# patflick/psac

Hardware: AMD Instinct MI355X
Metric: MChars/s SA+LCP build; rank-pair radix-sort HBM GB/s vs peak (higher is better)
Workload: dtype u64

## Files before the change

include/psacx.h:

```cpp
#ifndef PSACX_H
#define PSACX_H

#include <stddef.h>
#include <stdint.h>

#ifdef __cplusplus
extern "C" {
#endif

typedef struct psacx_ctx psacx_ctx;

enum {
    PSACX_OK = 0,
    PSACX_EINVAL = -1,
    PSACX_ERANGE = -2,
    PSACX_ENOMEM = -3,
    PSACX_EHIP = -4,
    PSACX_EDEVICE = -5,
    PSACX_ENOGPU = -6
};

enum {
    PSACX_LCP = 1u,
    PSACX_NO_FAST = 2u,
// ... 15 lines not shown
    uint32_t sigma;
    uint32_t bits_per_char;
    uint32_t k;
    uint32_t n_rounds;
    psacx_round rounds[PSACX_MAX_ROUNDS];
    double ms_total;
    double ms_alphabet, ms_kmer, ms_sort_hist, ms_sort_scatter, ms_rebucket, ms_isa_scatter,
           ms_gather, ms_compact, ms_rmq_build, ms_finalize;
    double ms_sort_scatter3, ms_sort_tilehist, ms_sort_scatter2;
    uint64_t scatter_launches[3];
    uint64_t scatter_records[3];
    uint64_t scatter_bytes[3];
    uint64_t hist_bytes;
    uint64_t workspace_bytes;
    uint64_t onew_passes;
    uint64_t heavy_rounds;
    uint64_t heavy_records;
    uint64_t light_records;
    uint64_t level_gathers;
    double ms_host[9];
    uint64_t locate_fetches[2];
    uint64_t rebucket_1w;
    uint64_t group_sort;
    uint64_t grid_cuts;
} psacx_stats;


#define PSACX_STREAM_DEFAULT ((void*)(intptr_t)-1)
int psacx_create(psacx_ctx** out, int device, void* stream);
void psacx_destroy(psacx_ctx* ctx);
const char* psacx_strerror(int code);
const char* psacx_last_hip_error(const psacx_ctx* ctx);
int psacx_trim(psacx_ctx* ctx);

enum {
    PSACX_OPT_RESET = 0, PSACX_OPT_FORCE_DIET, PSACX_OPT_DIET_CAP, PSACX_OPT_ONE_STAGE, PSACX_OPT_TIES_RADIX, PSACX_OPT_NO_ONE_WORD,
    PSACX_OPT_ONE_WORD_ALWAYS, PSACX_OPT_ONE_WORD_MIN, PSACX_OPT_WIDEN_LAST, PSACX_OPT_NO_DIGIT_BYTES, PSACX_OPT_NO_BUCKET_SORT,
    PSACX_OPT_ISA_UPDATE, PSACX_OPT_GATHER, PSACX_OPT_NO_HEAVY, PSACX_OPT_NO_WHOLE, PSACX_OPT_NO_LAZY_RANKS, PSACX_OPT_NO_EARLY_OUT,
    PSACX_OPT_NO_SPREAD_CURSORS, PSACX_OPT_LOCATE_SHAPE, PSACX_OPT_LOCATE_COUNT, PSACX_OPT_GENERIC_REBUCKET,
    PSACX_OPT_PLAIN_SIDE_KERNELS, PSACX_OPT_LSD_BUCKET_PASSES, PSACX_OPT_FIRST_LEAD, PSACX_OPT_LZ_SMALL_TILES,
    PSACX_OPT_GRID_CAP, PSACX_OPT_GROUP_COUNTING_ROUNDS, PSACX_OPT_MEMS_STOP, PSACX_OPT_KMISMATCH_STOP,
    PSACX_OPT_KEDIT_STOP,
    PSACX_OPT_COUNT
};
int psacx_configure(psacx_ctx* ctx, int option, uint64_t value);
int psacx_configure_from_env(psacx_ctx* ctx);
const char* psacx_debug_env(const char* name);

int psacx_construct_u32(psacx_ctx* ctx, const uint8_t* text, uint64_t n, uint32_t k,
                        uint32_t flags, uint32_t* SA, uint32_t* ISA, uint32_t* LCP);
int psacx_construct_u64(psacx_ctx* ctx, const uint8_t* text, uint64_t n, uint32_t k,
                        uint32_t flags, uint64_t* SA, uint64_t* ISA, uint64_t* LCP);
int psacx_construct_dev_u32(psacx_ctx* ctx, const uint8_t* d_text, uint64_t n, uint32_t k,
                            uint32_t flags, uint32_t* d_SA, uint32_t* d_ISA, uint32_t* d_LCP);
int psacx_construct_dev_u64(psacx_ctx* ctx, const uint8_t* d_text, uint64_t n, uint32_t k,
                            uint32_t flags, uint64_t* d_SA, uint64_t* d_ISA, uint64_t* d_LCP);

int psacx_construct_lc_u32(psacx_ctx* ctx, const uint8_t* text, uint64_t n, uint32_t k, uint32_t flags,
                           uint32_t* SA, uint32_t* ISA, uint32_t* LCP, uint8_t* Lc);
int psacx_construct_lc_u64(psacx_ctx* ctx, const uint8_t* text, uint64_t n, uint32_t k, uint32_t flags,
                           uint64_t* SA, uint64_t* ISA, uint64_t* LCP, uint8_t* Lc);
int psacx_construct_lc_dev_u32(psacx_ctx* ctx, const uint8_t* d_text, uint64_t n, uint32_t k, uint32_t flags,
                               uint32_t* d_SA, uint32_t* d_ISA, uint32_t* d_LCP, uint8_t* d_Lc);
int psacx_construct_lc_dev_u64(psacx_ctx* ctx, const uint8_t* d_text, uint64_t n, uint32_t k, uint32_t flags,
                               uint64_t* d_SA, uint64_t* d_ISA, uint64_t* d_LCP, uint8_t* d_Lc);

// ... 379 lines not shown
```

psac_amd/_lib.py:

```python
import ctypes as C
import os

_HERE = os.path.dirname(os.path.abspath(__file__))
LIB_PATH = os.path.join(_HERE, "lib", "libpsacx.so")

PSACX_LCP = 1
PSACX_NO_FAST = 2
PSACX_PROFILE = 4
PSACX_MAX_ROUNDS = 72
PSACX_MATCH_SUFFIXES = 1
PSACX_OVERLAP_WHOLE = 1
PSACX_REPEATS_RIGHT, PSACX_REPEATS_MAXIMAL, PSACX_REPEATS_SUPERMAXIMAL = 0, 1, 2
PSACX_MEMS_SUPER = 1
PSACX_KEDIT_BEST = 1

OPTIONS = {"reset": 0, "force_diet": 1, "diet_cap": 2, "one_stage": 3, "ties_radix": 4, "no_one_word": 5, "one_word_always": 6, "one_word_min": 7,
           "widen_last": 8, "no_digit_bytes": 9, "no_bucket_sort": 10, "isa_update": 11, "gather": 12, "no_heavy": 13, "no_whole": 14, "no_lazy_ranks": 15, "no_early_out": 16,
           "no_spread_cursors": 17, "locate_shape": 18, "locate_count": 19, "generic_rebucket": 20,
           "plain_side_kernels": 21, "lsd_bucket_passes": 22, "first_lead": 23, "lz_small_tiles": 24,
           "grid_cap": 25}
KERNEL_OPTIONS = {"group_counting_rounds": 26, "mems_stop": 27, "kmismatch_stop": 28, "kedit_stop": 29}
MULTI_OPTIONS = {"layout": 1, "slab": 2, "output_slack": 3, "trace": 4, "wire_piece": 5, "pieces": 6, "check_chunks": 7, "global_refine_sort": 8,
                 "one_stage": 9, "two_word": 10, "one_word": 11, "no_slices": 12, "slice_wide": 13, "slice_shape": 14}
MULTI_FORCE_WIRE, MULTI_NO_RCCL, MULTI_SHM = 1, 2, 4
ENV_KNOBS = bool(os.environ.get("PSACX_ENV_KNOBS"))
if ENV_KNOBS and os.environ.get("PSACX_LIB"):
    LIB_PATH = os.environ["PSACX_LIB"]

EXPORTS = [
    "psacx_create", "psacx_destroy", "psacx_strerror", "psacx_last_hip_error", "psacx_trim", "psacx_configure", "psacx_configure_from_env", "psacx_debug_env",
    "psacx_construct_u32", "psacx_construct_u64", "psacx_construct_dev_u32", "psacx_construct_dev_u64",
    "psacx_construct_gsa_u32", "psacx_construct_gsa_u64", "psacx_construct_gsa_dev_u32", "psacx_construct_gsa_dev_u64",
    "psacx_construct_lc_u32", "psacx_construct_lc_u64", "psacx_construct_lc_dev_u32", "psacx_construct_lc_dev_u64",
    "psacx_get_stats", "psacx_profile", "psacx_check_dev_u32", "psacx_check_dev_u64", "psacx_check_gsa_dev_u32", "psacx_check_gsa_dev_u64", "psacx_pair_sort_dev_u32", "psacx_pair_sort_dev_u64", "psacx_ansv_u32",
    "psacx_ansv_u64", "psacx_ansv_dev_u32", "psacx_ansv_dev_u64", "psacx_suffix_tree_u32", "psacx_suffix_tree_u64", "psacx_suffix_tree_dev_u32", "psacx_suffix_tree_dev_u64",
    "psacx_check_suffix_tree_dev_u32", "psacx_check_suffix_tree_dev_u64",
    "psacx_suffix_tree_gsa_u32", "psacx_suffix_tree_gsa_u64", "psacx_suffix_tree_gsa_dev_u32", "psacx_suffix_tree_gsa_dev_u64",
    "psacx_check_suffix_tree_gsa_dev_u32", "psacx_check_suffix_tree_gsa_dev_u64", "psacx_dev_alloc", "psacx_dev_free", "psacx_copy_h2d", "psacx_copy_d2h", "psacx_sync",
    "psacx_rand_dna", "psacx_synth_text_dev",
    "psacx_lookup_table_dev_u32", "psacx_lookup_table_dev_u64", "psacx_locate_dev_u32", "psacx_locate_dev_u64", "psacx_locate_u32", "psacx_locate_u64",
    "psacx_string_ends_dev", "psacx_lookup_table_gsa_dev_u32", "psacx_lookup_table_gsa_dev_u64", "psacx_locate_gsa_dev_u32", "psacx_locate_gsa_dev_u64",
    "psacx_locate_gsa_u32", "psacx_locate_gsa_u64", "psacx_occurrences_dev_u32", "psacx_occurrences_dev_u64",
    "psacx_match_dev_u32", "psacx_match_dev_u64", "psacx_match_gsa_dev_u32", "psacx_match_gsa_dev_u64",
    "psacx_match_u32", "psacx_match_u64", "psacx_match_gsa_u32", "psacx_match_gsa_u64",
# ... 18 lines not shown
    "psacx_multi_left_chars_dev_u32", "psacx_multi_left_chars_dev_u64", "psacx_multi_construct_lc_u32", "psacx_multi_construct_lc_u64",
    "psacx_multi_configure", "psacx_multi_configure_from_env", "psacx_multi_create_ex", "psacx_multi_create_rank_ex", "psacx_multi_get_memory", "psacx_multi_transport", "psacx_multi_get_wire", "psacx_multi_get_phases", "psacx_multi_last_form",
]


class Round(C.Structure):
    _fields_ = [("h", C.c_uint64), ("active", C.c_uint64), ("unfinished_buckets", C.c_uint64),
                ("unfinished_elements", C.c_uint64), ("sort_passes", C.c_uint32),
                ("sort_passes_skipped", C.c_uint32)]


class Stats(C.Structure):
    _fields_ = [("sigma", C.c_uint32), ("bits_per_char", C.c_uint32), ("k", C.c_uint32),
                ("n_rounds", C.c_uint32), ("rounds", Round * PSACX_MAX_ROUNDS),
                ("ms_total", C.c_double), ("ms_alphabet", C.c_double), ("ms_kmer", C.c_double),
                ("ms_sort_hist", C.c_double), ("ms_sort_scatter", C.c_double), ("ms_rebucket", C.c_double),
                ("ms_isa_scatter", C.c_double), ("ms_gather", C.c_double), ("ms_compact", C.c_double),
                ("ms_rmq_build", C.c_double), ("ms_finalize", C.c_double),
                ("ms_sort_scatter3", C.c_double), ("ms_sort_tilehist", C.c_double), ("ms_sort_scatter2", C.c_double),
                ("scatter_launches", C.c_uint64 * 3), ("scatter_records", C.c_uint64 * 3),
                ("scatter_bytes", C.c_uint64 * 3), ("hist_bytes", C.c_uint64), ("workspace_bytes", C.c_uint64), ("onew_passes", C.c_uint64),
                ("heavy_rounds", C.c_uint64), ("heavy_records", C.c_uint64), ("light_records", C.c_uint64), ("level_gathers", C.c_uint64),
                ("ms_host", C.c_double * 9), ("locate_fetches", C.c_uint64 * 2), ("rebucket_1w", C.c_uint64),
                ("group_sort", C.c_uint64), ("grid_cuts", C.c_uint64)]


class PsacxError(RuntimeError):
    def __init__(self, code, msg):
        RuntimeError.__init__(self, "psacx error %d: %s" % (code, msg))
        self.code = code


_lib = None


def load():
    global _lib
    if _lib is not None:
        return _lib
    if not os.path.exists(LIB_PATH):
        raise ImportError("libpsacx.so not built (%s); run `python -c 'import __graft_entry__ as g; g.build()'`"
                          % LIB_PATH)
    try:
        import torch
    except ImportError:
        pass
    lib = C.CDLL(LIB_PATH, mode=C.RTLD_GLOBAL)
# ... 150 lines not shown
```

psac_amd/csrc/dev_common.hpp:

```cpp
#pragma once
#include <hip/hip_runtime.h>
#include <stdint.h>

namespace psacx {

constexpr int WAVE = 64;

__device__ __forceinline__ unsigned lane_id() {
    return __builtin_amdgcn_mbcnt_hi(~0u, __builtin_amdgcn_mbcnt_lo(~0u, 0u));
}
__device__ __forceinline__ uint64_t lanemask_lt() {
    return (1ull << lane_id()) - 1ull;
}

template <typename T> __device__ __forceinline__ T shfl(T v, int src);
template <> __device__ __forceinline__ uint32_t shfl<uint32_t>(uint32_t v, int src) {
    return (uint32_t)__shfl((int)v, src, WAVE);
}
template <> __device__ __forceinline__ uint64_t shfl<uint64_t>(uint64_t v, int src) {
    uint32_t lo = (uint32_t)__shfl((int)(uint32_t)v, src, WAVE);
    uint32_t hi = (uint32_t)__shfl((int)(uint32_t)(v >> 32), src, WAVE);
    return ((uint64_t)hi << 32) | lo;
}
template <typename T> __device__ __forceinline__ T shfl_up(T v, int d);
// ... 13 lines not shown
    return (uint32_t)__shfl_xor((int)v, m, WAVE);
}
template <> __device__ __forceinline__ uint64_t shfl_xor<uint64_t>(uint64_t v, int m) {
    uint32_t lo = (uint32_t)__shfl_xor((int)(uint32_t)v, m, WAVE);
    uint32_t hi = (uint32_t)__shfl_xor((int)(uint32_t)(v >> 32), m, WAVE);
    return ((uint64_t)hi << 32) | lo;
}

__device__ __forceinline__ unsigned xcc_id() {
    return (unsigned)__builtin_amdgcn_s_getreg((3 << 11) | (0 << 6) | 20) & 7u;
}

__device__ __forceinline__ unsigned claim_tile(unsigned* qcnt, unsigned ntiles, unsigned chunk) {
    if (chunk == 0) return atomicAdd(qcnt, 1u);
    const unsigned x = xcc_id();
    for (unsigned r = 0; r < 8; ++r) {
        const unsigned q = (x + r) & 7u;
        const unsigned k = atomicAdd(&qcnt[q], 1u);
        const unsigned long long tile = ((unsigned long long)(k / chunk) * 8u + q) * chunk + k % chunk;
        if (tile < ntiles) return (unsigned)tile;
    }
    return ntiles;
}

struct OpSum {
    template <typename T> __device__ __forceinline__ T operator()(T a, T b) const { return a + b; }
};
struct OpMax {
    template <typename T> __device__ __forceinline__ T operator()(T a, T b) const { return a > b ? a : b; }
};
struct OpOr {
    template <typename T> __device__ __forceinline__ T operator()(T a, T b) const { return a | b; }
};
struct OpAnd {
    template <typename T> __device__ __forceinline__ T operator()(T a, T b) const { return a & b; }
};
struct OpMin {
    template <typename T> __device__ __forceinline__ T operator()(T a, T b) const { return a < b ? a : b; }
};

template <typename T, typename Op>
__device__ __forceinline__ T wave_reduce(T v, Op op) {
#pragma unroll
    for (int m = 32; m >= 1; m >>= 1) v = op(v, shfl_xor<T>(v, m));
    return v;
}
// ... 6 lines not shown
        T o = shfl_up<T>(v, d);
        if (lane >= (unsigned)d) v = op(o, v);
    }
    return v;
}

template <int BLOCK, typename T, typename Op>
__device__ __forceinline__ T block_scan_exclusive(T v, Op op, T identity, T* smem, T* total) {
    constexpr int NW = BLOCK / WAVE;
    const unsigned lane = lane_id();
    const unsigned wave = threadIdx.x / WAVE;
    T inc = wave_scan_inclusive<T>(v, op);
    if (lane == WAVE - 1) smem[wave] = inc;
    __syncthreads();
    T wprefix = identity;
    T tot = identity;
#pragma unroll
    for (int w = 0; w < NW; ++w) {
        T s = smem[w];
        if ((unsigned)w < wave) wprefix = op(wprefix, s);
        tot = op(tot, s);
    }
    T prev = shfl_up<T>(inc, 1);
    T excl = (lane == 0) ? wprefix : op(wprefix, prev);
    *total = tot;
    __syncthreads();
    return excl;
}

template <int BLOCK, typename T, typename Op>
__device__ __forceinline__ T block_reduce(T v, Op op, T* smem) {
    constexpr int NW = BLOCK / WAVE;
    v = wave_reduce<T>(v, op);
    if (lane_id() == 0) smem[threadIdx.x / WAVE] = v;
    __syncthreads();
    T r = smem[0];
#pragma unroll
    for (int w = 1; w < NW; ++w) r = op(r, smem[w]);
    __syncthreads();
    return r;
}

template <typename D> struct Desc;
template <> struct Desc<uint64_t> {
    static constexpr int SHIFT = 62;
    static constexpr uint64_t MASK = (1ull << 62) - 1ull;
// ... 160 lines not shown
```

psac_amd/csrc/engine.hpp:

```cpp
#pragma once
#include <hip/hip_runtime.h>

#include <algorithm>
#include <cstdio>
#include <cstdlib>
#include <cstring>
#include <condition_variable>
#include <functional>
#include <map>
#include <mutex>
#include <string>
#include <thread>
#include <sched.h>
#include <pthread.h>
#include <cctype>
#include <cstdio>
#include <vector>

#include "../../include/psacx.h"
#include "radix.hpp"
#include "sa_kernels.hpp"

namespace psacx {

// ... 7 lines not shown
namespace psacx { struct HostPool; }

namespace psacx {
struct Knobs {
    bool force_diet = false;
    uint64_t diet_cap = 0;
    bool one_stage = false;
    bool ties_radix = false;
    bool no_one_word = false;
    bool one_word_always = false;
    unsigned one_word_min = 24;
    int isa_update = 0;
    bool no_digit_bytes = false;
    bool no_bucket_sort = false;
    int gather = 0;
    bool no_heavy = false;
    bool no_early_out = false;
    bool no_lazy_ranks = false;
    bool no_whole = false;
    bool widen_last = false;
    bool no_spread_cursors = false;
    bool generic_rebucket = false;
    bool plain_side_kernels = false;
    bool lsd_bucket_passes = false;
    bool group_counting_rounds = false;
    unsigned first_lead = 0;
    bool lz_small_tiles = false;
    int locate_shape = 0;
    bool locate_count = false;
    unsigned mems_stop = 0;
    unsigned kedit_stop = 0;
    unsigned kmismatch_stop = 0;
    unsigned grid_cap = 0;
};

}

struct psacx_ctx {
    int device = 0;
    hipStream_t stream = nullptr;
    bool own_stream = false;
    char* slab = nullptr;
    size_t slab_bytes = 0;
    char* aux = nullptr;
    size_t aux_bytes = 0;
    char* pinned = nullptr;
// ... 942 lines not shown
            hipLaunchKernelGGL((top_digit_hist_kernel<uint64_t, BLOCK, ITEMS>), dim3((unsigned)ntiles), dim3(BLOCK), 0, c->stream, text, n, n_text, tab, ks, p0.tile_hist);
        else
            hipLaunchKernelGGL((top_digit_hist_waves_kernel<256>), dim3((unsigned)grid_for(c, ntiles * WAVE, 256, 5)), dim3(256), 0, c->stream, text, n, n_text, tab, ks,
                               ntiles, p0.tile_hist);
        PSACX_HIP(c, hipGetLastError());
    }
    {
        ProfScope ps(c, TC_SORT_TILEHIST);
        launch_pass_scans(c, p0, base0);
        PSACX_HIP(c, hipGetLastError());
    }
    PSACX_HIP(c, hipMemcpyAsync(sc.h_base, base0, RADIX * sizeof(unsigned long long), hipMemcpyDeviceToHost, c->stream));
    PSACX_HIP(c, hipStreamSynchronize(c->stream));
    unsigned long long* h_tabs = sc.h_base + (PIN_TABS - PIN_BASE) / sizeof(unsigned long long);
    for (int d = 0; d < RADIX; ++d) h_tabs[d] = sc.h_base[d];
    h_tabs[RADIX] = n;
    OneWordLayout lay = onew_layout<TILE>(h_tabs, ntiles);
    if (lay.need > sc.desc_bytes || lay.vtiles >= (1ull << 31)) return PSACX_RETRY_1W;
    if (view_out && dig && tie_bytes && !c->knobs.lsd_bucket_passes) lay = onew_group_layout<TILE>(lay, n, low, sc.desc_bytes);
    unsigned long long* const h_word = sc.h_base + (PIN_GROUP_WORD - PIN_BASE) / sizeof(unsigned long long);
    {
        ProfScope ps(c, TC_KMER);
        PSACX_HIP(c, hipMemsetAsync(scratch, 0, 256, c->stream));
        hipLaunchKernelGGL((key_scatter1w_kernel<BLOCK, ITEMS>), dim3((unsigned)ntiles), dim3(BLOCK), 0, c->stream, text, n, n_text, tab, ks, pad ? k0 : a, (int)(lo1 + low),
                           base0, p0.tile_hist, p0.slab_tot, p0.counter, sort_chunk_for(n, true), p0.slab_tiles, lo1 | (sfield << 16), (uint64_t)0,
                           (uint8_t*)nullptr, 0, pad);
        PSACX_HIP(c, hipGetLastError());
    }
    uint64_t* cur = nullptr;
    if (pad) PSACX_TRY(onew_bucket_passes(c, scratch, h_tabs, lay, k0, a, sa_out, sfield, low, lo1, n, &cur, view_out, dig, pad, tie_bytes, h_word));
    else PSACX_TRY(onew_bucket_passes(c, scratch, h_tabs, lay, a, k0, sa_out, sfield, low, lo1, n, &cur, view_out, dig, 0, tie_bytes, h_word));
    *s1 = cur;
    if (rs) { rs->sort_passes = (uint32_t)((low + RADIX_BITS - 1) / RADIX_BITS + 1); rs->sort_passes_skipped = 0; }
    return PSACX_OK;
}

}
```

psac_amd/csrc/psacx_abi.hip:

```cpp
#include "engine.hpp"
#include "query_calls.hpp"

namespace psacx {
int construct_dev_u32(psacx_ctx*, const uint8_t*, uint64_t, uint32_t, uint32_t, uint32_t*, uint32_t*, uint32_t*);
int construct_dev_u64(psacx_ctx*, const uint8_t*, uint64_t, uint32_t, uint32_t, uint64_t*, uint64_t*, uint64_t*);
int construct_host_u32(psacx_ctx*, const uint8_t*, uint64_t, uint32_t, uint32_t, uint32_t*, uint32_t*, uint32_t*);
int construct_gsa_host_u32(psacx_ctx*, const uint8_t*, uint64_t, const uint64_t*, uint64_t, uint32_t, uint32_t, uint32_t*, uint32_t*, uint32_t*);
int construct_gsa_dev_u32(psacx_ctx*, const uint8_t*, uint64_t, const uint64_t*, uint64_t, uint32_t, uint32_t, uint32_t*, uint32_t*, uint32_t*);
int construct_gsa_host_u64(psacx_ctx*, const uint8_t*, uint64_t, const uint64_t*, uint64_t, uint32_t, uint32_t, uint64_t*, uint64_t*, uint64_t*);
int construct_gsa_dev_u64(psacx_ctx*, const uint8_t*, uint64_t, const uint64_t*, uint64_t, uint32_t, uint32_t, uint64_t*, uint64_t*, uint64_t*);
int construct_lc_host_u32(psacx_ctx*, const uint8_t*, uint64_t, uint32_t, uint32_t, uint32_t*, uint32_t*, uint32_t*, uint8_t*);
int construct_lc_host_u64(psacx_ctx*, const uint8_t*, uint64_t, uint32_t, uint32_t, uint64_t*, uint64_t*, uint64_t*, uint8_t*);
int construct_lc_dev_u32(psacx_ctx*, const uint8_t*, uint64_t, uint32_t, uint32_t, uint32_t*, uint32_t*, uint32_t*, uint8_t*);
int construct_lc_dev_u64(psacx_ctx*, const uint8_t*, uint64_t, uint32_t, uint32_t, uint64_t*, uint64_t*, uint64_t*, uint8_t*);
int construct_host_u64(psacx_ctx*, const uint8_t*, uint64_t, uint32_t, uint32_t, uint64_t*, uint64_t*, uint64_t*);
int pair_sort_dev_u32(psacx_ctx*, uint32_t*, uint32_t*, uint32_t*, uint64_t, uint32_t);
int pair_sort_dev_u64(psacx_ctx*, uint64_t*, uint64_t*, uint64_t*, uint64_t, uint32_t);
int check_dev_u32(psacx_ctx*, const uint8_t*, uint64_t, const uint32_t*, const uint32_t*, const uint32_t*, uint64_t*);
int check_dev_u64(psacx_ctx*, const uint8_t*, uint64_t, const uint64_t*, const uint64_t*, const uint64_t*, uint64_t*);
int check_gsa_dev_u32(psacx_ctx*, const uint8_t*, uint64_t, const uint64_t*, uint64_t, const uint32_t*, const uint32_t*, const uint32_t*, uint64_t*);
int check_gsa_dev_u64(psacx_ctx*, const uint8_t*, uint64_t, const uint64_t*, uint64_t, const uint64_t*, const uint64_t*, const uint64_t*, uint64_t*);
int synth_text_dev(psacx_ctx*, uint8_t*, uint64_t, uint64_t, int, uint64_t, uint64_t);
int suffix_tree_host_u32(psacx_ctx*, const uint8_t*, uint64_t, const uint32_t*, const uint32_t*, uint64_t*, uint32_t*);
int suffix_tree_host_u64(psacx_ctx*, const uint8_t*, uint64_t, const uint64_t*, const uint64_t*, uint64_t*, uint32_t*);
// ... 84 lines not shown
    switch (option) {
    case PSACX_OPT_RESET: k = psacx::Knobs(); return PSACX_OK;
    case PSACX_OPT_FORCE_DIET: k.force_diet = value != 0; return PSACX_OK;
    case PSACX_OPT_DIET_CAP: k.diet_cap = value; return PSACX_OK;
    case PSACX_OPT_ONE_STAGE: k.one_stage = value != 0; return PSACX_OK;
    case PSACX_OPT_TIES_RADIX: k.ties_radix = value != 0; return PSACX_OK;
    case PSACX_OPT_NO_ONE_WORD: k.no_one_word = value != 0; return PSACX_OK;
    case PSACX_OPT_ONE_WORD_ALWAYS: k.one_word_always = value != 0; return PSACX_OK;
    case PSACX_OPT_ONE_WORD_MIN: if (value > 62) return PSACX_EINVAL; k.one_word_min = value ? (unsigned)std::max<uint64_t>(16, value) : 24u; return PSACX_OK;
    case PSACX_OPT_WIDEN_LAST: k.widen_last = value != 0; return PSACX_OK;
    case PSACX_OPT_NO_DIGIT_BYTES: k.no_digit_bytes = value != 0; return PSACX_OK;
    case PSACX_OPT_NO_BUCKET_SORT: k.no_bucket_sort = value != 0; return PSACX_OK;
    case PSACX_OPT_ISA_UPDATE: if (value > 2) return PSACX_EINVAL; k.isa_update = (int)value; return PSACX_OK;
    case PSACX_OPT_GATHER: if (value > 2) return PSACX_EINVAL; k.gather = (int)value; return PSACX_OK;
    case PSACX_OPT_NO_HEAVY: k.no_heavy = value != 0; return PSACX_OK;
    case PSACX_OPT_NO_WHOLE: k.no_whole = value != 0; return PSACX_OK;
    case PSACX_OPT_NO_LAZY_RANKS: k.no_lazy_ranks = value != 0; return PSACX_OK;
    case PSACX_OPT_NO_EARLY_OUT: k.no_early_out = value != 0; return PSACX_OK;
    case PSACX_OPT_NO_SPREAD_CURSORS: k.no_spread_cursors = value != 0; return PSACX_OK;
    case PSACX_OPT_LOCATE_SHAPE: if (value > 2) return PSACX_EINVAL; k.locate_shape = (int)value; return PSACX_OK;
    case PSACX_OPT_LOCATE_COUNT: k.locate_count = value != 0; return PSACX_OK;
    case PSACX_OPT_GENERIC_REBUCKET: k.generic_rebucket = value != 0; return PSACX_OK;
    case PSACX_OPT_PLAIN_SIDE_KERNELS: k.plain_side_kernels = value != 0; return PSACX_OK;
    case PSACX_OPT_LSD_BUCKET_PASSES: k.lsd_bucket_passes = value != 0; return PSACX_OK;
    case PSACX_OPT_GROUP_COUNTING_ROUNDS: k.group_counting_rounds = value != 0; return PSACX_OK;
    case PSACX_OPT_LZ_SMALL_TILES: k.lz_small_tiles = value != 0; return PSACX_OK;
    case PSACX_OPT_GRID_CAP: if (value > 65535) return PSACX_EINVAL; k.grid_cap = (unsigned)value; return PSACX_OK;
    case PSACX_OPT_MEMS_STOP: if (value > 3) return PSACX_EINVAL; k.mems_stop = (unsigned)value; return PSACX_OK;
    case PSACX_OPT_KMISMATCH_STOP: if (value > 2) return PSACX_EINVAL; k.kmismatch_stop = (unsigned)value; return PSACX_OK;
    case PSACX_OPT_KEDIT_STOP: if (value > 3) return PSACX_EINVAL; k.kedit_stop = (unsigned)value; return PSACX_OK;
    case PSACX_OPT_FIRST_LEAD: if (value > 64) return PSACX_EINVAL; k.first_lead = (unsigned)value; return PSACX_OK;
    default: return PSACX_EINVAL;
    }
}

const char* psacx_debug_env(const char* name) { return name ? getenv(name) : nullptr; }

int psacx_configure_from_env(psacx_ctx* c) {
    if (!c) return PSACX_EINVAL;
    static const struct { const char* name; int option; } flags[] = {
        {"PSACX_FORCE_DIET", PSACX_OPT_FORCE_DIET}, {"PSACX_ONE_STAGE", PSACX_OPT_ONE_STAGE}, {"PSACX_TIES_RADIX", PSACX_OPT_TIES_RADIX},
        {"PSACX_NO_ONE_WORD", PSACX_OPT_NO_ONE_WORD}, {"PSACX_ONE_WORD_ALWAYS", PSACX_OPT_ONE_WORD_ALWAYS}, {"PSACX_WIDEN_LAST", PSACX_OPT_WIDEN_LAST},
        {"PSACX_NO_DIGIT_BYTES", PSACX_OPT_NO_DIGIT_BYTES}, {"PSACX_NO_BUCKET_SORT", PSACX_OPT_NO_BUCKET_SORT}, {"PSACX_NO_HEAVY", PSACX_OPT_NO_HEAVY},
        {"PSACX_NO_WHOLE", PSACX_OPT_NO_WHOLE}, {"PSACX_NO_LAZY_RANKS", PSACX_OPT_NO_LAZY_RANKS},
        {"PSACX_NO_EARLY_OUT", PSACX_OPT_NO_EARLY_OUT}, {"PSACX_NO_SPREAD_CURSORS", PSACX_OPT_NO_SPREAD_CURSORS},
        {"PSACX_LOCATE_COUNT", PSACX_OPT_LOCATE_COUNT}, {"PSACX_GENERIC_REBUCKET", PSACX_OPT_GENERIC_REBUCKET},
        {"PSACX_PLAIN_SIDE_KERNELS", PSACX_OPT_PLAIN_SIDE_KERNELS}, {"PSACX_LSD_BUCKET_PASSES", PSACX_OPT_LSD_BUCKET_PASSES},
        {"PSACX_LZ_SMALL_TILES", PSACX_OPT_LZ_SMALL_TILES}, {"PSACX_GROUP_COUNTING_ROUNDS", PSACX_OPT_GROUP_COUNTING_ROUNDS}};
    (void)psacx_configure(c, PSACX_OPT_RESET, 0);
    for (const auto& f : flags) if (psacx_debug_env(f.name)) (void)psacx_configure(c, f.option, 1);
    if (const char* e = psacx_debug_env("PSACX_DIET_CAP")) (void)psacx_configure(c, PSACX_OPT_DIET_CAP, strtoull(e, nullptr, 10));
    if (const char* e = psacx_debug_env("PSACX_FIRST_LEAD")) (void)psacx_configure(c, PSACX_OPT_FIRST_LEAD, strtoull(e, nullptr, 10));
    if (const char* e = psacx_debug_env("PSACX_GRID_CAP")) (void)psacx_configure(c, PSACX_OPT_GRID_CAP, strtoull(e, nullptr, 10));
    if (const char* e = psacx_debug_env("PSACX_MEMS_STOP")) (void)psacx_configure(c, PSACX_OPT_MEMS_STOP, strtoull(e, nullptr, 10));
    if (const char* e = psacx_debug_env("PSACX_KMISMATCH_STOP")) (void)psacx_configure(c, PSACX_OPT_KMISMATCH_STOP, strtoull(e, nullptr, 10));
    if (const char* e = psacx_debug_env("PSACX_KEDIT_STOP")) (void)psacx_configure(c, PSACX_OPT_KEDIT_STOP, strtoull(e, nullptr, 10));
    if (const char* e = psacx_debug_env("PSACX_ONE_WORD_MIN")) (void)psacx_configure(c, PSACX_OPT_ONE_WORD_MIN, strtoull(e, nullptr, 10));
    if (const char* e = psacx_debug_env("PSACX_ISA_UPDATE")) (void)psacx_configure(c, PSACX_OPT_ISA_UPDATE, e[0] == 's' ? 1 : 2);
    if (const char* e = psacx_debug_env("PSACX_LOCATE_SHAPE")) (void)psacx_configure(c, PSACX_OPT_LOCATE_SHAPE, e[0] == 'g' ? 2 : 1);
    if (const char* e = psacx_debug_env("PSACX_GATHER")) (void)psacx_configure(c, PSACX_OPT_GATHER, e[0] == 'f' ? 1 : 2);
    return PSACX_OK;
}

int psacx_trim(psacx_ctx* c) {
    if (!c) return PSACX_EINVAL;
    PSACX_HIP(c, hipSetDevice(c->device));
    PSACX_HIP(c, hipStreamSynchronize(c->stream));
    if (c->slab) { PSACX_HIP(c, hipFree(c->slab)); c->slab = nullptr; c->slab_bytes = 0; }
    if (c->aux) { PSACX_HIP(c, hipFree(c->aux)); c->aux = nullptr; c->aux_bytes = 0; }
    if (c->io) { PSACX_HIP(c, hipFree(c->io)); c->io = nullptr; c->io_bytes = 0; }
    if (c->dstage) { PSACX_HIP(c, hipFree(c->dstage)); c->dstage = nullptr; }
// ... 173 lines not shown
```

psac_amd/csrc/radix.hpp:

```cpp
#pragma once
#include <type_traits>
#include "dev_common.hpp"
#include "sort_scratch.hpp"
#include "group_rank.hpp"

namespace psacx {


struct PassPlan {
    int n_pass;
    int word[MAX_PASSES];
    int shift[MAX_PASSES];
};

inline PassPlan make_plan(int bits1, int bits2, int lo1 = 0) {
    PassPlan p;
    p.n_pass = 0;
    for (int w = 1; w >= 0; --w) {
        const int lo = w ? 0 : lo1;
        const int per = ((w ? bits2 : bits1) - lo + RADIX_BITS - 1) / RADIX_BITS;
        for (int i = 0; i < per; ++i) { p.word[p.n_pass] = w; p.shift[p.n_pass] = lo + i * RADIX_BITS; p.n_pass++; }
    }
    return p;
}
// ... 63 lines not shown
__device__ __forceinline__ uint64_t match_any8(unsigned d, bool valid) {
    uint32_t lo = 0, hi = 0;
#pragma unroll
    for (int b = 0; b < RADIX_BITS; ++b) {
        int x = __builtin_amdgcn_sbfe((int)d, (unsigned)b, 1u);
        asm("" : "+v"(x));
        const uint64_t bal = __ballot(x != 0);
        lo = __builtin_amdgcn_bitop3_b32(lo, (uint32_t)bal, (uint32_t)x, 0xF6);
        hi = __builtin_amdgcn_bitop3_b32(hi, (uint32_t)(bal >> 32), (uint32_t)x, 0xF6);
    }
    return ~(((uint64_t)hi << 32) | lo) & __ballot(valid);
}

template <typename T, int TILE, int NW> struct ScatterShared {
    T stage[TILE];
    uint8_t sdig[TILE];
    unsigned wcnt[NW * RADIX];
    unsigned bstart[RADIX];
    T goff[RADIX];
    unsigned scan_tmp[NW + 1];
    unsigned s_tile;
};

template <typename T, typename D, int BLOCK, int ITEMS, bool FULL, bool LB, bool EXT = false, bool NOKO = false, int VN = 0, int CLSB = sizeof(T), bool DNEXT3 = false>
__device__ __forceinline__ void radix_scatter_tile(
    ScatterShared<T, BLOCK * ITEMS, BLOCK / WAVE>& sh, const unsigned tile, const unsigned count,
    const T* __restrict__ kd_in, const T* __restrict__ ko_in, const T* __restrict__ v_in,
    T* __restrict__ kd_out, T* __restrict__ ko_out, T* __restrict__ v_out, int shift,
    const unsigned long long* __restrict__ digit_base, D* __restrict__ desc, unsigned* __restrict__ err,
    unsigned long long* __restrict__ dbg, const uint64_t spec, const uint64_t spec_n,
    const unsigned* __restrict__ tile_excl, const unsigned long long* __restrict__ slab_excl,
    const T* __restrict__ dsrc = nullptr, const unsigned slab_tiles = SLAB_TILES, const uint64_t voff = 0, const unsigned pack = 0,
    const T (*kd_made)[ITEMS] = nullptr, uint8_t* __restrict__ dnext = nullptr, const int dnext_shift = 0, const uint64_t out_pad = 0,
    const int dnext_ko = 0) {
    constexpr int TILE = BLOCK * ITEMS;
    constexpr int NW = BLOCK / WAVE;
    constexpr bool ONEW_IN = VN == 8 || VN == 9;
    constexpr bool ONEW_OUT = VN == 7 || VN == 8 || VN == 10;
    constexpr bool ONEW_MAKE = VN == 7 || VN == 10;
    const unsigned sfield = (ONEW_MAKE || VN == 9) ? (((pack >> 16) & 255u) ? ((pack >> 16) & 255u) : 32u) : 0u;
    T* const stage = sh.stage;
    uint8_t* const sdig = sh.sdig;
    unsigned* const wcnt = sh.wcnt;
    unsigned* const bstart = sh.bstart;
    T* const goff = sh.goff;
    unsigned* const scan_tmp = sh.scan_tmp;

    const unsigned tid = threadIdx.x;
    const unsigned lane = lane_id();
    const unsigned wave = tid / WAVE;
    const bool stamp = dbg != nullptr && (tile & 63u) == 0 && tid == 0;
    unsigned long long* mydbg = dbg + (size_t)(tile >> 6) * 8;
    if (stamp) mydbg[0] = __builtin_amdgcn_s_memtime();
    const uint64_t base = (uint64_t)tile * TILE;

    const T* __restrict__ pkd = kd_in + base;
    const T* __restrict__ pko = ko_in + base;
    const T* __restrict__ pv = v_in ? v_in + base : nullptr;
    constexpr bool LATE_EXCL = NOKO && VN != 0;
    uint64_t pre_excl = 0;
    if (!LATE_EXCL && !LB && tid < RADIX)
        pre_excl = (uint64_t)tile_excl[(uint64_t)tile * RADIX + tid] + (uint64_t)slab_excl[(uint64_t)(tile / slab_tiles) * RADIX + tid] +
                   (uint64_t)digit_base[tid];
    typedef typename std::conditional<(VN != 0) && sizeof(T) == 8, uint32_t, T>::type PV;
    T kd[ITEMS], ko[NOKO ? 1 : ITEMS];
    PV vv[ITEMS];
    unsigned char cls[EXT ? ITEMS : 1];
    const unsigned wbase = wave * (WAVE * ITEMS) + lane;
    if (EXT) {
        const T* __restrict__ pd = dsrc + base;
        const unsigned char* __restrict__ pb = reinterpret_cast<const unsigned char*>(dsrc) + base;
#pragma unroll
// ... 48 lines not shown
        const unsigned prior = __hip_atomic_load(&mycnt[d], __ATOMIC_RELAXED, __HIP_MEMORY_SCOPE_WAVEFRONT);
        const unsigned below = __builtin_amdgcn_mbcnt_hi((unsigned)(m >> 32), __builtin_amdgcn_mbcnt_lo((unsigned)m, 0u));
        if (valid && below == 0)
            __hip_atomic_fetch_add(&mycnt[d], (unsigned)__builtin_popcountll(m), __ATOMIC_RELAXED, __HIP_MEMORY_SCOPE_WAVEFRONT);
        rank[i] = prior + below;
    }
    if (LATE_EXCL && !LB && tid < RADIX)
        pre_excl = (uint64_t)tile_excl[(uint64_t)tile * RADIX + tid] + (uint64_t)slab_excl[(uint64_t)(tile / slab_tiles) * RADIX + tid] +
                   (uint64_t)digit_base[tid];
    __syncthreads();
    if (stamp) mydbg[1] = __builtin_amdgcn_s_memtime();

    unsigned tot = 0;
    if (tid < RADIX) {
#pragma unroll
        for (int w = 0; w < NW; ++w) {
            const unsigned c = wcnt[w * RADIX + tid];
            wcnt[w * RADIX + tid] = tot;
            tot += c;
        }
        if (LB) desc_store<D>(desc + (uint64_t)tile * RADIX + tid, tile == 0 ? 2u : 1u, (D)tot);
    }
    unsigned tile_total;
    unsigned bs = block_scan_exclusive<BLOCK, unsigned>(tid < RADIX ? tot : 0u, OpSum(), 0u, scan_tmp, &tile_total);
    if (stamp) mydbg[2] = __builtin_amdgcn_s_memtime();
    if (tid < RADIX) {
        bstart[tid] = bs;
        uint64_t excl = 0;
        if (!LB) {
            excl = pre_excl;
        } else if (tile != 0) {
            long long t = (long long)tile - 1;
            const D* dp = desc + tid;
            while (t >= 0) {
                D d0 = desc_load<D>(dp + (uint64_t)t * RADIX);
                D d1 = t > 0 ? desc_load<D>(dp + (uint64_t)(t - 1) * RADIX) : (D)0;
                if ((d0 >> Desc<D>::SHIFT) == 0) d0 = desc_wait<D>(dp + (uint64_t)t * RADIX, err);
                excl += (uint64_t)(d0 & Desc<D>::MASK);
                if ((d0 >> Desc<D>::SHIFT) == 2u) break;
                if (t == 0) break;
                if ((d1 >> Desc<D>::SHIFT) == 0) d1 = desc_wait<D>(dp + (uint64_t)(t - 1) * RADIX, err);
                excl += (uint64_t)(d1 & Desc<D>::MASK);
                if ((d1 >> Desc<D>::SHIFT) == 2u) break;
                t -= 2;
            }
            desc_store<D>(desc + (uint64_t)tile * RADIX + tid, 2u, (D)(excl + tot));
        }
// ... 743 lines not shown
```

psac_amd/csrc/sa_kernels.hpp:

```cpp
#pragma once
#ifndef RB_WAVES_ATTR
#define RB_WAVES_ATTR
#endif
#ifndef RB_ABLATE
#define RB_ABLATE 0
#endif
#include <type_traits>
#include "dev_common.hpp"
#include "rebucket_1w_math.hpp"

namespace psacx {

constexpr int RADIX_P = 256;

struct CodeTable { uint16_t c[256]; };

template <typename T>
__device__ __forceinline__ void key_summary_add(unsigned long long* partials, T or1, T and1, T or2, T and2) {
    __shared__ unsigned long long red[4][16];
    or1 = wave_reduce<T>(or1, OpOr()); and1 = wave_reduce<T>(and1, OpAnd());
    or2 = wave_reduce<T>(or2, OpOr()); and2 = wave_reduce<T>(and2, OpAnd());
    const unsigned wave = threadIdx.x / WAVE, nw = (blockDim.x + WAVE - 1) / WAVE;
    const unsigned long long hi = ~(unsigned long long)(T)~(T)0;
    if (lane_id() == 0) {
// ... 435 lines not shown
            if (rec >= ks.spec) {
                const unsigned o = (unsigned)(rel + (long long)p) * lc;
                const unsigned m = o >> 5, sft = o & 31u;
                const uint64_t x = ((uint64_t)stream[m] << 32) | stream[m + 1];
                const uint64_t r = (x << sft) | (((uint64_t)stream[m + 2] << sft) >> 32);
                w1 = r >> (64u - wbits);
            } else if (rec < n) {
                const uint64_t i0 = record_suffix(rec, ks.spec, n);
                for (unsigned t = 0; t < ks.c1; ++t) w1 = (T)(w1 << lc) | (T)((i0 + t < n_text) ? tab.c[text[i0 + t]] : 0);
            }
            kd[i] = rec < n ? w1 : (T)0;
        }
    }
    __syncthreads();
    const uint64_t remain = n - base;
    if (remain >= (uint64_t)TILE)
        radix_scatter_tile<T, unsigned, BLOCK, ITEMS, true, false, false, true, 10>(sh, tile, (unsigned)TILE, nullptr, nullptr, nullptr, out, nullptr, nullptr, shift,
                                                                                   digit_base, nullptr, nullptr, nullptr, ks.spec, ks.spec ? n : (uint64_t)0, tile_excl, slab_excl, nullptr,
                                                                                   slab_tiles, voff, lo1, &kd, dnext, dnext_shift, out_pad);
    else
        radix_scatter_tile<T, unsigned, BLOCK, ITEMS, false, false, false, true, 10>(sh, tile, (unsigned)remain, nullptr, nullptr, nullptr, out, nullptr, nullptr, shift,
                                                                                    digit_base, nullptr, nullptr, nullptr, ks.spec, ks.spec ? n : (uint64_t)0, tile_excl, slab_excl, nullptr,
                                                                                    slab_tiles, voff, lo1, &kd, dnext, dnext_shift, out_pad);
}

template <typename T>
__device__ __forceinline__ unsigned window_lcp(T x1, T x2, T y1, T y2, const KeyShape& ks) {
    if (x1 != y1) return (clz_t<T>((T)(x1 ^ y1)) - (unsigned)(sizeof(T) * 8 - ks.c1 * ks.lc)) / ks.lc;
    if (x2 != y2) return ks.c1 + (clz_t<T>((T)(x2 ^ y2)) - (unsigned)(sizeof(T) * 8 - ks.c2 * ks.lc)) / ks.lc;
    return ks.c1 + ks.c2;
}

template <bool GSA, typename T>
__device__ __forceinline__ uint64_t first_round_len(uint64_t ng, T sa, T w1, T w2, const KeyShape& ks) {
    if (!GSA) return ng - (uint64_t)sa;
    if (ks.c2 && w2 != 0) return ks.c1 + ks.c2 - ctz_t<T>(w2) / ks.lc;
    return w1 != 0 ? ks.c1 - ctz_t<T>(w1) / ks.lc : 0;
}

template <typename T> struct Boundary {
    uint64_t off;
    uint64_t base;
    int has_prev, has_next;
    T prev1, prev2, prev3;
    T next1, next2, next3;
};
// ... 2172 lines not shown
```

Before: 30980.

## Add persistent key-scatter kernel that prefetches next tile's text while scattering

```diff
diff --git a/include/psacx.h b/include/psacx.h
--- a/include/psacx.h
+++ b/include/psacx.h
@@ -61,6 +61,7 @@
     uint64_t locate_fetches[2];
     uint64_t rebucket_1w;
     uint64_t group_sort;
+    uint64_t key_scatter_waves;
     uint64_t grid_cuts;
 } psacx_stats;
 
@@ -80,7 +81,8 @@
     PSACX_OPT_PLAIN_SIDE_KERNELS, PSACX_OPT_LSD_BUCKET_PASSES, PSACX_OPT_FIRST_LEAD, PSACX_OPT_LZ_SMALL_TILES,
     PSACX_OPT_GRID_CAP, PSACX_OPT_GROUP_COUNTING_ROUNDS, PSACX_OPT_MEMS_STOP, PSACX_OPT_KMISMATCH_STOP,
     PSACX_OPT_KEDIT_STOP,
-    PSACX_OPT_COUNT
+    PSACX_OPT_COUNT = PSACX_OPT_KEDIT_STOP + 2,
+    PSACX_OPT_PLAIN_KEY_SCATTER = PSACX_OPT_KEDIT_STOP + 1
 };
 int psacx_configure(psacx_ctx* ctx, int option, uint64_t value);
 int psacx_configure_from_env(psacx_ctx* ctx);
diff --git a/psac_amd/_lib.py b/psac_amd/_lib.py
--- a/psac_amd/_lib.py
+++ b/psac_amd/_lib.py
@@ -19,7 +19,7 @@
            "no_spread_cursors": 17, "locate_shape": 18, "locate_count": 19, "generic_rebucket": 20,
            "plain_side_kernels": 21, "lsd_bucket_passes": 22, "first_lead": 23, "lz_small_tiles": 24,
            "grid_cap": 25}
-KERNEL_OPTIONS = {"group_counting_rounds": 26, "mems_stop": 27, "kmismatch_stop": 28, "kedit_stop": 29}
+KERNEL_OPTIONS = {"group_counting_rounds": 26, "mems_stop": 27, "kmismatch_stop": 28, "kedit_stop": 29, "plain_key_scatter": 30}
 MULTI_OPTIONS = {"layout": 1, "slab": 2, "output_slack": 3, "trace": 4, "wire_piece": 5, "pieces": 6, "check_chunks": 7, "global_refine_sort": 8,
                  "one_stage": 9, "two_word": 10, "one_word": 11, "no_slices": 12, "slice_wide": 13, "slice_shape": 14}
 MULTI_FORCE_WIRE, MULTI_NO_RCCL, MULTI_SHM = 1, 2, 4
@@ -84,7 +84,7 @@
                 ("scatter_bytes", C.c_uint64 * 3), ("hist_bytes", C.c_uint64), ("workspace_bytes", C.c_uint64), ("onew_passes", C.c_uint64),
                 ("heavy_rounds", C.c_uint64), ("heavy_records", C.c_uint64), ("light_records", C.c_uint64), ("level_gathers", C.c_uint64),
                 ("ms_host", C.c_double * 9), ("locate_fetches", C.c_uint64 * 2), ("rebucket_1w", C.c_uint64),
-                ("group_sort", C.c_uint64), ("grid_cuts", C.c_uint64)]
+                ("group_sort", C.c_uint64), ("key_scatter_waves", C.c_uint64), ("grid_cuts", C.c_uint64)]
 
 
 class PsacxError(RuntimeError):
diff --git a/psac_amd/csrc/dev_common.hpp b/psac_amd/csrc/dev_common.hpp
--- a/psac_amd/csrc/dev_common.hpp
+++ b/psac_amd/csrc/dev_common.hpp
@@ -59,6 +59,21 @@
     }
     return ntiles;
 }
+__device__ __forceinline__ unsigned claim_begin(unsigned* qcnt, unsigned chunk, unsigned x) {
+    unsigned zero = 0;
+    asm volatile("" : "+v"(zero));
+    return atomicAdd(&qcnt[(chunk ? x : 0u) + zero], 1u);
+}
+__device__ __forceinline__ unsigned claim_end(unsigned* qcnt, unsigned ntiles, unsigned chunk, unsigned x, unsigned k) {
+    if (chunk == 0) return k < ntiles ? k : ntiles;
+    for (unsigned r = 0; r < 8; ++r) {
+        const unsigned q = (x + r) & 7u;
+        if (r) k = atomicAdd(&qcnt[q], 1u);
+        const unsigned long long tile = ((unsigned long long)(k / chunk) * 8u + q) * chunk + k % chunk;
+        if (tile < ntiles) return (unsigned)tile;
+    }
+    return ntiles;
+}
 
 struct OpSum {
     template <typename T> __device__ __forceinline__ T operator()(T a, T b) const { return a + b; }
@@ -111,6 +126,33 @@
         tot = op(tot, s);
     }
     T prev = shfl_up<T>(inc, 1);
+    T excl = (lane == 0) ? wprefix : op(wprefix, prev);
+    *total = tot;
+    __syncthreads();
+    return excl;
+}
+
+template <int BLOCK, typename T, typename Op>
+__device__ __forceinline__ T block_scan_exclusive_at(T v, Op op, T identity, T* smem, T* total, unsigned lane, unsigned wave) {
+    static_assert(sizeof(T) == 4, "one ds_bpermute per step");
+    constexpr int NW = BLOCK / WAVE;
+    T inc = v;
+#pragma unroll
+    for (int d = 1; d < WAVE; d <<= 1) {
+        const T o = (T)__builtin_amdgcn_ds_bpermute((int)((lane - (unsigned)d) << 2), (int)inc);
+        if (lane >= (unsigned)d) inc = op(o, inc);
+    }
+    if (lane == WAVE - 1) smem[wave] = inc;
+    __syncthreads();
+    T wprefix = identity;
+    T tot = identity;
+#pragma unroll
+    for (int w = 0; w < NW; ++w) {
+        T s = smem[w];
+        if ((unsigned)w < wave) wprefix = op(wprefix, s);
+        tot = op(tot, s);
+    }
+    const T prev = (T)__builtin_amdgcn_ds_bpermute((int)((lane - 1u) << 2), (int)inc);
     T excl = (lane == 0) ? wprefix : op(wprefix, prev);
     *total = tot;
     __syncthreads();
diff --git a/psac_amd/csrc/engine.hpp b/psac_amd/csrc/engine.hpp
--- a/psac_amd/csrc/engine.hpp
+++ b/psac_amd/csrc/engine.hpp
@@ -53,6 +53,7 @@
     bool no_spread_cursors = false;
     bool generic_rebucket = false;
     bool plain_side_kernels = false;
+    bool plain_key_scatter = false;
     bool lsd_bucket_passes = false;
     bool group_counting_rounds = false;
     unsigned first_lead = 0;
@@ -1041,9 +1042,15 @@
     {
         ProfScope ps(c, TC_KMER);
         PSACX_HIP(c, hipMemsetAsync(scratch, 0, 256, c->stream));
-        hipLaunchKernelGGL((key_scatter1w_kernel<BLOCK, ITEMS>), dim3((unsigned)ntiles), dim3(BLOCK), 0, c->stream, text, n, n_text, tab, ks, pad ? k0 : a, (int)(lo1 + low),
-                           base0, p0.tile_hist, p0.slab_tot, p0.counter, sort_chunk_for(n, true), p0.slab_tiles, lo1 | (sfield << 16), (uint64_t)0,
-                           (uint8_t*)nullptr, 0, pad);
+        c->stats.key_scatter_waves = c->knobs.plain_key_scatter ? 0 : 1;
+        if (c->knobs.plain_key_scatter)
+            hipLaunchKernelGGL((key_scatter1w_kernel<BLOCK, ITEMS>), dim3((unsigned)ntiles), dim3(BLOCK), 0, c->stream, text, n, n_text, tab, ks, pad ? k0 : a, (int)(lo1 + low),
+                               base0, p0.tile_hist, p0.slab_tot, p0.counter, sort_chunk_for(n, true), p0.slab_tiles, lo1 | (sfield << 16), (uint64_t)0,
+                               (uint8_t*)nullptr, 0, pad);
+        else
+            hipLaunchKernelGGL((key_scatter1w_waves_kernel<BLOCK, ITEMS>), dim3((unsigned)grid_for(c, ntiles * BLOCK, BLOCK, 3)), dim3(BLOCK), 0, c->stream, text, n, n_text, tab,
+                               ks, pad ? k0 : a, (int)(lo1 + low), base0, p0.tile_hist, p0.slab_tot, p0.counter, sort_chunk_for(n, true), p0.slab_tiles,
+                               lo1 | (sfield << 16), (unsigned)ntiles, (uint64_t)0, (uint8_t*)nullptr, 0, pad);
         PSACX_HIP(c, hipGetLastError());
     }
     uint64_t* cur = nullptr;
diff --git a/psac_amd/csrc/psacx_abi.hip b/psac_amd/csrc/psacx_abi.hip
--- a/psac_amd/csrc/psacx_abi.hip
+++ b/psac_amd/csrc/psacx_abi.hip
@@ -130,6 +130,7 @@
     case PSACX_OPT_LOCATE_COUNT: k.locate_count = value != 0; return PSACX_OK;
     case PSACX_OPT_GENERIC_REBUCKET: k.generic_rebucket = value != 0; return PSACX_OK;
     case PSACX_OPT_PLAIN_SIDE_KERNELS: k.plain_side_kernels = value != 0; return PSACX_OK;
+    case PSACX_OPT_PLAIN_KEY_SCATTER: k.plain_key_scatter = value != 0; return PSACX_OK;
     case PSACX_OPT_LSD_BUCKET_PASSES: k.lsd_bucket_passes = value != 0; return PSACX_OK;
     case PSACX_OPT_GROUP_COUNTING_ROUNDS: k.group_counting_rounds = value != 0; return PSACX_OK;
     case PSACX_OPT_LZ_SMALL_TILES: k.lz_small_tiles = value != 0; return PSACX_OK;
@@ -154,7 +155,8 @@
         {"PSACX_NO_EARLY_OUT", PSACX_OPT_NO_EARLY_OUT}, {"PSACX_NO_SPREAD_CURSORS", PSACX_OPT_NO_SPREAD_CURSORS},
         {"PSACX_LOCATE_COUNT", PSACX_OPT_LOCATE_COUNT}, {"PSACX_GENERIC_REBUCKET", PSACX_OPT_GENERIC_REBUCKET},
         {"PSACX_PLAIN_SIDE_KERNELS", PSACX_OPT_PLAIN_SIDE_KERNELS}, {"PSACX_LSD_BUCKET_PASSES", PSACX_OPT_LSD_BUCKET_PASSES},
-        {"PSACX_LZ_SMALL_TILES", PSACX_OPT_LZ_SMALL_TILES}, {"PSACX_GROUP_COUNTING_ROUNDS", PSACX_OPT_GROUP_COUNTING_ROUNDS}};
+        {"PSACX_LZ_SMALL_TILES", PSACX_OPT_LZ_SMALL_TILES}, {"PSACX_GROUP_COUNTING_ROUNDS", PSACX_OPT_GROUP_COUNTING_ROUNDS},
+        {"PSACX_PLAIN_KEY_SCATTER", PSACX_OPT_PLAIN_KEY_SCATTER}};
     (void)psacx_configure(c, PSACX_OPT_RESET, 0);
     for (const auto& f : flags) if (psacx_debug_env(f.name)) (void)psacx_configure(c, f.option, 1);
     if (const char* e = psacx_debug_env("PSACX_DIET_CAP")) (void)psacx_configure(c, PSACX_OPT_DIET_CAP, strtoull(e, nullptr, 10));
diff --git a/psac_amd/csrc/radix.hpp b/psac_amd/csrc/radix.hpp
--- a/psac_amd/csrc/radix.hpp
+++ b/psac_amd/csrc/radix.hpp
@@ -109,7 +109,8 @@
     unsigned s_tile;
 };
 
-template <typename T, typename D, int BLOCK, int ITEMS, bool FULL, bool LB, bool EXT = false, bool NOKO = false, int VN = 0, int CLSB = sizeof(T), bool DNEXT3 = false>
+template <typename T, typename D, int BLOCK, int ITEMS, bool FULL, bool LB, bool EXT = false, bool NOKO = false, int VN = 0, int CLSB = sizeof(T), bool DNEXT3 = false,
+          bool TRIPS = false>
 __device__ __forceinline__ void radix_scatter_tile(
     ScatterShared<T, BLOCK * ITEMS, BLOCK / WAVE>& sh, const unsigned tile, const unsigned count,
     const T* __restrict__ kd_in, const T* __restrict__ ko_in, const T* __restrict__ v_in,
@@ -133,8 +134,10 @@
     T* const goff = sh.goff;
     unsigned* const scan_tmp = sh.scan_tmp;
 
-    const unsigned tid = threadIdx.x;
-    const unsigned lane = lane_id();
+    unsigned tid_ = threadIdx.x, lane_ = lane_id();
+    if constexpr (TRIPS) asm volatile("" : "+v"(tid_), "+v"(lane_));
+    const unsigned tid = tid_;
+    const unsigned lane = lane_;
     const unsigned wave = tid / WAVE;
     const bool stamp = dbg != nullptr && (tile & 63u) == 0 && tid == 0;
     unsigned long long* mydbg = dbg + (size_t)(tile >> 6) * 8;
@@ -229,7 +232,9 @@
         if (LB) desc_store<D>(desc + (uint64_t)tile * RADIX + tid, tile == 0 ? 2u : 1u, (D)tot);
     }
     unsigned tile_total;
-    unsigned bs = block_scan_exclusive<BLOCK, unsigned>(tid < RADIX ? tot : 0u, OpSum(), 0u, scan_tmp, &tile_total);
+    unsigned bs;
+    if constexpr (TRIPS) bs = block_scan_exclusive_at<BLOCK, unsigned>(tid < RADIX ? tot : 0u, OpSum(), 0u, scan_tmp, &tile_total, lane, wave);
+    else bs = block_scan_exclusive<BLOCK, unsigned>(tid < RADIX ? tot : 0u, OpSum(), 0u, scan_tmp, &tile_total);
     if (stamp) mydbg[2] = __builtin_amdgcn_s_memtime();
     if (tid < RADIX) {
         bstart[tid] = bs;
diff --git a/psac_amd/csrc/sa_kernels.hpp b/psac_amd/csrc/sa_kernels.hpp
--- a/psac_amd/csrc/sa_kernels.hpp
+++ b/psac_amd/csrc/sa_kernels.hpp
@@ -481,6 +481,143 @@
         radix_scatter_tile<T, unsigned, BLOCK, ITEMS, false, false, false, true, 10>(sh, tile, (unsigned)remain, nullptr, nullptr, nullptr, out, nullptr, nullptr, shift,
                                                                                     digit_base, nullptr, nullptr, nullptr, ks.spec, ks.spec ? n : (uint64_t)0, tile_excl, slab_excl, nullptr,
                                                                                     slab_tiles, voff, lo1, &kd, dnext, dnext_shift, out_pad);
+}
+
+template <int BLOCK, int ITEMS>
+__global__ __launch_bounds__(BLOCK, 6) void key_scatter1w_waves_kernel(const uint8_t* __restrict__ text, uint64_t n, uint64_t n_text, CodeTable tab, KeyShape ks,
+                                                                       uint64_t* __restrict__ out, int shift, const unsigned long long* __restrict__ digit_base,
+                                                                       const unsigned* __restrict__ tile_excl, const unsigned long long* __restrict__ slab_excl,
+                                                                       unsigned* __restrict__ tile_counter, unsigned chunk, unsigned slab_tiles, unsigned lo1,
+                                                                       unsigned ntiles, uint64_t voff = 0, uint8_t* __restrict__ dnext = nullptr, int dnext_shift = 0,
+                                                                       uint64_t out_pad = 0) {
+    typedef uint64_t T;
+    constexpr int TILE = BLOCK * ITEMS;
+    constexpr int NW = BLOCK / WAVE;
+    constexpr int HALO = 2 * 64 + 8 + 16;
+    __shared__ ScatterShared<T, TILE, NW> sh;
+    __shared__ uint16_t ctab[256];
+    __shared__ unsigned s_last;
+    static_assert(sizeof(uint32_t) * ((TILE + HALO) * 8 / 32 + 4) <= sizeof(sh.stage), "the packed codes of the tile live in the stage until the words are cut out");
+    static_assert((TILE + 64 + 16 + 15) / 16 <= BLOCK, "a thread stages at most one 16-byte piece of the tile's text: it holds the next tile's in four registers");
+    uint32_t* const stream = reinterpret_cast<uint32_t*>(sh.stage);
+    uint16_t* const stream16 = reinterpret_cast<uint16_t*>(sh.stage);
+    const unsigned xcd = xcc_id();
+    const unsigned partial = (n % TILE) ? ntiles - 1 : ntiles;
+    auto claimed = [&](unsigned ch, unsigned x, unsigned ticket) -> unsigned {
+        unsigned t = claim_end(tile_counter, ntiles, ch, x, ticket);
+        if (t == partial && t < ntiles) {
+            s_last = 1;
+            t = claim_end(tile_counter, ntiles, ch, x, claim_begin(tile_counter, ch, x));
+        }
+        return t;
+    };
+    if (threadIdx.x == 0) {
+        s_last = 0;
+        sh.s_tile = claimed(chunk, xcd, claim_begin(tile_counter, chunk, xcd));
+    }
+    for (int i = threadIdx.x; i < NW * RADIX; i += BLOCK) sh.wcnt[i] = 0;
+    for (int i = threadIdx.x; i < 256; i += BLOCK) ctab[i] = tab.c[i];
+    __syncthreads();
+    unsigned tile = sh.s_tile;
+    const unsigned lc = ks.lc;
+    const unsigned need = TILE + ks.c1 + 16;
+    const bool aligned_ptr = (reinterpret_cast<uintptr_t>(text) & 15u) == 0;
+    auto window = [&](unsigned t) -> uint64_t {
+        const uint64_t base = (uint64_t)t * TILE;
+        return ((base > ks.spec ? base : ks.spec) - ks.spec) & ~15ull;
+    };
+    auto fetch = [&](unsigned t, unsigned tid, uint4& x) -> bool {
+        if (t >= ntiles || tid * 16u >= need || !aligned_ptr) return false;
+        const uint64_t g0 = window(t) + (uint64_t)tid * 16u;
+        if (g0 + 16 > n_text) return false;
+        x = *reinterpret_cast<const uint4*>(text + g0);
+        return true;
+    };
+    auto write_stream = [&](unsigned tid, uint64_t a_lo, bool fast, const uint4& held) {
+        if (tid * 16u < need) {
+            const unsigned v = tid;
+            const uint64_t g0 = a_lo + (uint64_t)v * 16u;
+            uint16_t cd[16];
+            if (fast) {
+                const unsigned wds[4] = {held.x, held.y, held.z, held.w};
+#pragma unroll
+                for (int b = 0; b < 16; ++b) cd[b] = ctab[(wds[b >> 2] >> ((b & 3) * 8)) & 255u];
+            } else {
+#pragma unroll
+                for (int b = 0; b < 16; ++b) cd[b] = (g0 + b) < n_text ? ctab[text[g0 + b]] : (uint16_t)0;
+            }
+            uint32_t acc = 0;
+            unsigned nb = 0, h = lc * v;
+#pragma unroll
+            for (int b = 0; b < 16; ++b) {
+                acc = (acc << lc) | cd[b];
+                nb += lc;
+                if (nb >= 16) { nb -= 16; stream16[(h++) ^ 1u] = (uint16_t)(acc >> nb); }
+            }
+        }
+    };
+    auto cut_out = [&](unsigned tid, unsigned lane, uint64_t base, uint64_t a_lo, T (&kd)[ITEMS]) {
+        const unsigned wbase = (tid / WAVE) * (WAVE * ITEMS) + lane;
+        const unsigned wbits = ks.c1 * lc;
+        const long long rel = (long long)base - (long long)ks.spec - (long long)a_lo;
+#pragma unroll
+        for (int i = 0; i < ITEMS; ++i) {
+            const unsigned p = wbase + (unsigned)i * WAVE;
+            const uint64_t rec = base + p;
+            T w1 = 0;
+            if (rec >= ks.spec) {
+                const unsigned o = (unsigned)(rel + (long long)p) * lc;
+                const unsigned m = o >> 5, sft = o & 31u;
+                const uint64_t x2 = ((uint64_t)stream[m] << 32) | stream[m + 1];
+                const uint64_t r = (x2 << sft) | (((uint64_t)stream[m + 2] << sft) >> 32);
+                w1 = r >> (64u - wbits);
+            } else if (rec < n) {
+                const uint64_t i0 = record_suffix(rec, ks.spec, n);
+                for (unsigned t = 0; t < ks.c1; ++t) w1 = (T)(w1 << lc) | (T)((i0 + t < n_text) ? tab.c[text[i0 + t]] : 0);
+            }
+            kd[i] = rec < n ? w1 : (T)0;
+        }
+    };
+    uint4 held = make_uint4(0, 0, 0, 0);
+    bool fast = fetch(tile, threadIdx.x, held);
+    asm volatile("" : : "v"(held.x), "v"(held.y), "v"(held.z), "v"(held.w));
+    while (tile < ntiles) {
+        unsigned tid = threadIdx.x, lane = lane_id(), x = xcd, chunk_t = chunk, slab_tiles_t = slab_tiles;
+        uint64_t spec_n = ks.spec ? n : (uint64_t)0;
+        asm volatile("" : "+v"(tid), "+v"(lane), "+s"(x), "+s"(chunk_t), "+s"(slab_tiles_t), "+s"(spec_n));
+        asm volatile("" : : "v"(held.x), "v"(held.y), "v"(held.z), "v"(held.w));
+        unsigned ticket = 0;
+        if (tid == 0) ticket = claim_begin(tile_counter, chunk_t, x);
+        const uint64_t base = (uint64_t)tile * TILE;
+        const uint64_t a_lo = window(tile);
+        write_stream(tid, a_lo, fast, held);
+        __syncthreads();
+        T kd[ITEMS];
+        cut_out(tid, lane, base, a_lo, kd);
+        if (tid == 0) sh.s_tile = claimed(chunk_t, x, ticket);
+        __syncthreads();
+        const unsigned next = sh.s_tile;
+        fast = fetch(next, tid, held);
+        radix_scatter_tile<T, unsigned, BLOCK, ITEMS, true, false, false, true, 10, sizeof(T), false, true>(
+            sh, tile, (unsigned)TILE, nullptr, nullptr, nullptr, out, nullptr, nullptr, shift, digit_base, nullptr, nullptr, nullptr, ks.spec, spec_n,
+            tile_excl, slab_excl, nullptr, slab_tiles_t, voff, lo1, &kd, dnext, dnext_shift, out_pad);
+        for (int i = tid; i < NW * RADIX; i += BLOCK) sh.wcnt[i] = 0;
+        __syncthreads();
+        tile = next;
+    }
+    if (s_last) {
+        const uint64_t base = (uint64_t)partial * TILE;
+        const uint64_t a_lo = window(partial);
+        fast = fetch(partial, threadIdx.x, held);
+        write_stream(threadIdx.x, a_lo, fast, held);
+        __syncthreads();
+        T kd[ITEMS];
+        cut_out(threadIdx.x, lane_id(), base, a_lo, kd);
+        __syncthreads();
+        radix_scatter_tile<T, unsigned, BLOCK, ITEMS, false, false, false, true, 10>(sh, partial, (unsigned)(n - base), nullptr, nullptr, nullptr, out, nullptr, nullptr, shift,
+                                                                                    digit_base, nullptr, nullptr, nullptr, ks.spec, ks.spec ? n : (uint64_t)0, tile_excl, slab_excl, nullptr,
+                                                                                    slab_tiles, voff, lo1, &kd, dnext, dnext_shift, out_pad);
+    }
 }
 
 template <typename T>
```

Result: no change. 31290 (median of 6 runs) (+1.0%).
